# Samsung/tf-fast-rnnt

Hardware: AMD Instinct MI355X
Metric: rnnt_loss_pruned_fwd_bwd_throughput (higher is better)
Workload: dtype f32; 1 GPU; c3: rnnt_loss_pruned fwd+bwd step, B=32/GPU T=1000 S=200 C=500 s_range=5, regular, full boundary, first pass rnnt_loss_simple; global_batch=32, am_pruned=broadcast view

## Files before the change

### tf-fast-rnnt_amd/csrc/ftr_common.h

```cpp
#pragma once
#include <hip/hip_runtime.h>
#include <stdint.h>
#include <stdio.h>
#include <stdarg.h>
#include "../../include/ftr.h"

namespace ftr {

void set_error(const char* fmt, ...);
void clear_error();

inline int check_launch(const char* what) {
  hipError_t e = hipGetLastError();
  if (e != hipSuccess) {
    set_error("%s: launch failed: %s", what, hipGetErrorString(e));
    return FTR_ERR_LAUNCH;
  }
  return FTR_OK;
}

__global__ void zero_words_kernel(uint32_t* __restrict__ p, size_t n);
__global__ void copy_words_kernel(uint32_t* __restrict__ dst, const uint32_t* __restrict__ src, size_t n);
inline int zero_words(void* p, size_t n_words, hipStream_t st, const char* what) {
  if (n_words == 0) return FTR_OK;
// ... 43 lines not shown
  v = fmaxf(v, dpp_take<0x112, 0xf, 0xf>(ninf, v));
  v = fmaxf(v, dpp_take<0x114, 0xf, 0xe>(ninf, v));
  v = fmaxf(v, dpp_take<0x118, 0xf, 0xc>(ninf, v));
  v = fmaxf(v, dpp_take<0x142, 0xa, 0xf>(ninf, v));
  v = fmaxf(v, dpp_take<0x143, 0xc, 0xf>(ninf, v));
  return __builtin_bit_cast(float, __builtin_amdgcn_readlane(__builtin_bit_cast(int, v), 63));
}

struct Shift { float cx2, cy2; };
__device__ __forceinline__ bool shift_sample_ok(float v) { return v > -1.0e4f && v < 1.0e4f; }
template <bool MOD>
__device__ __forceinline__ Shift shift_from_sums(float sumx, float nx, float sumy, float ny, int Sn, int Tn) {
  const float steps = MOD ? (float)(Tn - 1) : (float)(Sn - 1 + Tn - 1);
  float f = steps > 0.0f ? (float)(Sn - 1) / steps : 0.5f;
  f = fminf(fmaxf(f, 1.0e-3f), 1.0f - 1.0e-3f);
  const float mx = nx > 0.0f ? sumx / nx : 0.0f, my = ny > 0.0f ? sumy / ny : 0.0f;
  Shift s;
  s.cx2 = mx * kLog2e - __builtin_amdgcn_logf(f);
  s.cy2 = my * kLog2e - __builtin_amdgcn_logf(1.0f - f);
  return s;
}
template <bool MOD>
__device__ __forceinline__ double shift_total(const Shift s, int Sn, int Tn) {
  const int nx = Sn - 1, ny = MOD ? (Tn - 1) - (Sn - 1) : (Tn - 1);
  return (double)nx * (double)s.cx2 + (double)ny * (double)s.cy2;
}

struct Bound { int sb, tb, se, te; };
__device__ __forceinline__ Bound load_boundary(const int32_t* __restrict__ boundary, int b, int S, int T) {
  Bound r;
  if (boundary) {
    r.sb = max(boundary[4 * b + 0], 0); r.tb = max(boundary[4 * b + 1], 0);
    r.se = min(boundary[4 * b + 2], S); r.te = min(boundary[4 * b + 3], T);
  } else { r.sb = 0; r.tb = 0; r.se = S; r.te = T; }
  return r;
}

__device__ __forceinline__ float softplus(float v) { return fmaxf(v, 0.0f) + log1pf(expf(-fabsf(v))); }
__device__ __forceinline__ void hat_logprobs(float xb, float xs, float Z, bool sym_is_blank, float* vx, float* vy) {
  *vy = -softplus(-xb);
  *vx = sym_is_blank ? -INFINITY : (xs - Z) - softplus(xb);
}
__device__ __forceinline__ void hat_sigmoids(float xb, float* sp, float* sn) {
  const float e = expf(-fabsf(xb)), big = 1.0f / (1.0f + e), small = e / (1.0f + e);
  *sp = xb >= 0.0f ? big : small;
  *sn = xb >= 0.0f ? small : big;
}

}

namespace ftr {
int mi_plain_fwd(const float* px, const float* py, const int32_t* boundary, float* p, float* ans, int B, int S, int T, int modified, hipStream_t st);
int mi_plain_bwd(const float* px, const float* py, const int32_t* boundary, const float* p, float* p_grad, float* px_grad, float* py_grad, float* ans_grad, int overwrite, int B, int S, int T, int modified, hipStream_t st);
int mi_bidir_fwd(const float* px, const float* py, const int32_t* boundary, float* ws, size_t ws_floats, int flags, float* ans, int B, int S, int T, int modified, hipStream_t st);
int mi_bidir_bwd(const int32_t* boundary, const float* ws, size_t ws_floats, int flags, float* px_grad, float* py_grad, float* ans_grad, int overwrite, int B, int S, int T, int modified, hipStream_t st, const float* ans = nullptr, float* loss_out = nullptr, int loss_code = 0);
int mi_bidir_ws_init(float* ws, size_t ws_floats, int B, int S, int T, hipStream_t st);
int mi_bidir_status(const float* ws, size_t ws_floats, int B, int S, int T, int* status_host, long long* dirty_host, hipStream_t st);
size_t mi_bidir_workspace_floats(int B, int S, int T);
size_t mi_bidir_handoff_floats(int B, int S, int T);
size_t mi_viterbi_workspace_bytes(int B, int S, int T);
int mi_viterbi(const float* px, const float* py, const int32_t* boundary, void* ws, size_t ws_bytes, float* score, int32_t* frames, int B, int S, int T, int modified, hipStream_t st);
int cummin_i32(const int32_t* in, int32_t* out, int rows, int cols, hipStream_t st);
int prune_ranges(const float* px_grad, const float* py_grad, const int32_t* boundary, int32_t* ranges, int32_t* s_begin, int B, int S, int T, int T1, int r, hipStream_t st);
int do_pruning(const float* am, const float* lm, const int32_t* ranges, float* am_p, float* lm_p, int B, int T, int S1, int C, int r, hipStream_t st);
size_t do_pruning_bwd_workspace_bytes(int B, int T, int S1, int C, int r);
int do_pruning_bwd_ws(const float* g_am_p, const float* g_lm_p, const int32_t* ranges, float* d_am, float* d_lm, int B, int T, int S1, int C, int r, void* ws, size_t ws_bytes, hipStream_t st);
int do_pruning_bwd(const float* g_am_p, const float* g_lm_p, const int32_t* ranges, float* d_am, float* d_lm, int B, int T, int S1, int C, int r, hipStream_t st);
int pruned_logprobs_fwd(const float* logits, const int32_t* symbols, const int32_t* ranges, const int32_t* boundary, int blank, double delay_penalty, float* lse, float* px, float* py, int B, int T, int S, int C, int r, int modified, int hat, hipStream_t st);
int pruned_logprobs_bwd(const float* logits, const int32_t* symbols, const int32_t* ranges, const int32_t* boundary, int blank, const float* lse, const float* gpx, const float* gpy, Scale scale, float* glogits, int B, int T, int S, int C, int r, int modified, int hat, hipStream_t st);
int simple_rowmax_exp(const float* x, float* probs, float* rowmax, float* rowsum, const float* dotvec, float* dot, size_t rows, int C, hipStream_t st);
int simple_rowmax_exp_pair(const float* x1, float* probs1, float* rowmax1, size_t rows1, const float* x2, float* probs2, float* rowmax2, size_t rows2, int C, hipStream_t st);
int simple_rowdot(const float* x, const float* v, float* dot, size_t rows, int C, hipStream_t st);
size_t simple_colsum_workspace_floats(size_t rows, int C);
int simple_colsum_weighted(const float* x, const float* w, float* out, float* ws, size_t ws_floats, size_t rows, int C, hipStream_t st);
int simple_logprobs_fwd(const float* am, const float* lm, const int32_t* symbols, const float* prod, const float* am_max, const float* lm_max, const int32_t* boundary, int blank, double delay_penalty, const float* lmonly_norm, const float* amonly_norm, const float* ulog, float cs, float ls, float as, float* px, float* py, int B, int T, int S, int C, int modified, hipStream_t st);
int simple_logprobs_bwd_w(const float* gpx, const float* gpy, Scale scale, const float* prod, const int32_t* boundary, float* W, float* rsx, float* rsy, float cs, int B, int T, int S, int modified, hipStream_t st);
int simple_logprobs_bwd_am(const float* gpx, const float* gpy, Scale scale, const float* damp, const float* am_probs, const int32_t* symbols, const int32_t* boundary, int blank, float kdir, const float* uvec, const float* amdot, float as, float* Rout, float* d_am, int B, int T, int S, int C, int modified, hipStream_t st);
int simple_logprobs_bwd_lm(const float* dlmp, const float* lm_probs, const int32_t* symbols, const float* rsx, const float* rsy, int blank, float kdir, const float* arow, const float* invsum, const float* gu, float* d_lm, int B, int S, int C, hipStream_t st);
int simple_fused_supported(int C);
int simple_fused_bwd_supported(int T, int C);
int normalizer_gemm(int kind, const float* x, const float* y, float* out, int B, int T, int S1, int C, hipStream_t st);
int normalizer_gemm_choice(int kind, int B, int T, int S1, int C, int* solution, float* us, float* us_default, int* candidates);
int normalizer_gemm_set_choice(int kind, int B, int T, int S1, int C, int solution);
int simple_fused_fwd(const float* am, const float* lm, const int32_t* symbols, const float* am_probs, const float* lm_probs, const float* am_max, const float* lm_max, const int32_t* boundary, int blank, double delay_penalty, const float* lmonly_norm, const float* amonly_norm, const float* ulog, float cs, float ls, float as, float* px, float* py, float* prod_out, int B, int T, int S, int C, int modified, hipStream_t st);
int simple_fused_bwd_am(const float* gpx, const float* gpy, Scale scale, const float* prod, const float* lm_probs, const float* am_probs, const int32_t* symbols, const int32_t* boundary, int blank, float cs, float kdir, const float* uvec, const float* amdot, float as, float* Rout, float* d_am, int B, int T, int S, int C, int modified, hipStream_t st);
int negated_reduce(const float* ans, int B, int reduction, float* out, hipStream_t st);
int lse_rows(const float* logits, float* lse, size_t rows, int C, int blank, int hat, hipStream_t st);
int mi_band_supported(int T, int S, int r);
int band_ranges_check(const int32_t* ranges, const int32_t* boundary, int* flags, int B, int T, int r, hipStream_t st);
int band_gather(const float* logits, const int32_t* symbols, const int32_t* ranges, const int32_t* boundary, const float* lse, int blank, double delay_penalty, float* pxb, float* pyb, int B, int T, int S, int C, int r, int modified, int hat, hipStream_t st);
size_t mi_band_workspace_floats(int B, int T, int S, int r);
int mi_band_seg_supported(int T, int S, int r);
size_t mi_band_seg_workspace_floats(int B, int T, int S, int r);
int mi_band_seg(const float* pxb, const float* pyb, const int32_t* ranges, const int32_t* boundary, float* ws, size_t ws_floats, float* ans, float* gxb, float* gyb, int B, int T, int S, int r, int modified, hipStream_t st);
int mi_band(const float* pxb, const float* pyb, const int32_t* ranges, const int32_t* boundary, float* ws, size_t ws_floats, float* ans, float* gxb, float* gyb, int B, int T, int S, int r, int modified, hipStream_t st);
int band_grad_banded(const float* logits, const int32_t* symbols, const int32_t* ranges, const int32_t* boundary, int blank, const float* lse, const float* gxb, const float* gyb, Scale scale, float* glogits, int B, int T, int S, int C, int r, int modified, int hat, hipStream_t st);
int selftest(hipStream_t st, int* result_dev);
int debug_stamps(unsigned long long* out16);
int debug_trace(unsigned long long* out, int n);
}
```

### tf-fast-rnnt_amd/csrc/normalizer_gemm.hip

```cpp
#define ROCBLAS_BETA_FEATURES_API 1
#define ROCBLAS_NO_DEPRECATED_WARNINGS 1
#include <rocblas/rocblas.h>

#include <cstdlib>
#include <cstring>
#include <map>
#include <mutex>
#include <tuple>
#include <vector>

#include "ftr_common.h"

namespace ftr {
namespace {

struct Shape {
  int ta, tb, m, n, k, lda, ldb, ldc, batch, device;
  long long sa, sb, sc;
  bool operator<(const Shape& o) const {
    return std::tie(ta, tb, m, n, k, lda, ldb, ldc, batch, device, sa, sb, sc) <
           std::tie(o.ta, o.tb, o.m, o.n, o.k, o.lda, o.ldb, o.ldc, o.batch, o.device, o.sa, o.sb, o.sc);
  }
};
struct Choice {
  int seen = 0;
  bool tuned = false;
  int solution = 0;
  float us = 0.f, us_default = 0.f;
  int candidates = 0;
};

std::mutex g_mu;
std::map<int, rocblas_handle> g_handles;
std::map<Shape, Choice> g_choices;

int tune_mode() {
  const char* e = getenv("FTR_GEMM_TUNE");
  if (!e || !strcmp(e, "second") || !strcmp(e, "auto")) return 2;
  if (!strcmp(e, "first")) return 1;
  return 0;
}

rocblas_status run(rocblas_handle h, const Shape& s, const float* A, const float* B, float* C, rocblas_gemm_algo algo, int sol) {
  const float one = 1.0f, zero = 0.0f;
  return rocblas_gemm_strided_batched_ex(h, (rocblas_operation)s.ta, (rocblas_operation)s.tb, s.m, s.n, s.k, &one, A,
                                         rocblas_datatype_f32_r, s.lda, s.sa, B, rocblas_datatype_f32_r, s.ldb, s.sb, &zero, C,
                                         rocblas_datatype_f32_r, s.ldc, s.sc, C, rocblas_datatype_f32_r, s.ldc, s.sc, s.batch,
                                         rocblas_datatype_f32_r, algo, sol, rocblas_gemm_flags_none);
}

void tune(rocblas_handle h, const Shape& s, const float* A, const float* B, float* C, hipStream_t st, Choice& ch) {
  const float one = 1.0f, zero = 0.0f;
  rocblas_int n = 0;
  auto query = [&](rocblas_int* list, rocblas_int* size) {
    return rocblas_gemm_strided_batched_ex_get_solutions(h, (rocblas_operation)s.ta, (rocblas_operation)s.tb, s.m, s.n, s.k, &one, A,
                                                         rocblas_datatype_f32_r, s.lda, s.sa, B, rocblas_datatype_f32_r, s.ldb, s.sb,
                                                         &zero, C, rocblas_datatype_f32_r, s.ldc, s.sc, C, rocblas_datatype_f32_r,
                                                         s.ldc, s.sc, s.batch, rocblas_datatype_f32_r, rocblas_gemm_algo_solution_index,
                                                         rocblas_gemm_flags_none, list, size);
  };
  ch.tuned = true;
  if (query(nullptr, &n) != rocblas_status_success || n <= 0) return;
  std::vector<rocblas_int> sols((size_t)n);
  if (query(sols.data(), &n) != rocblas_status_success) return;
  hipEvent_t e0, e1;
  if (hipEventCreate(&e0) != hipSuccess) return;
  if (hipEventCreate(&e1) != hipSuccess) { (void)hipEventDestroy(e0); return; }
  auto time_one = [&](rocblas_gemm_algo algo, int sol, int reps) -> float {
    if (run(h, s, A, B, C, algo, sol) != rocblas_status_success) return -1.f;
    (void)hipEventRecord(e0, st);
    for (int i = 0; i < reps; ++i)
      if (run(h, s, A, B, C, algo, sol) != rocblas_status_success) return -1.f;
    (void)hipEventRecord(e1, st);
    if (hipEventSynchronize(e1) != hipSuccess) return -1.f;
    float ms = 0.f;
    (void)hipEventElapsedTime(&ms, e0, e1);
    return 1e3f * ms / reps;
  };
  const float def = time_one(rocblas_gemm_algo_standard, 0, 3);
  std::vector<std::pair<float, int>> timed;
  float fastest = 1e30f;
  for (int i = 0; i < n; ++i) {
    const float t = time_one(rocblas_gemm_algo_solution_index, sols[(size_t)i], 1);
    if (t > 0.f) { timed.emplace_back(t, sols[(size_t)i]); fastest = t < fastest ? t : fastest; }
  }
  float best = def > 0.f ? def : 1e30f;
  int best_sol = 0;
  for (const auto& p : timed) {
    if (p.first > 1.15f * fastest) continue;
    const float t = time_one(rocblas_gemm_algo_solution_index, p.second, 4);
    if (t > 0.f && t < 0.97f * best) { best = t; best_sol = p.second; }
  }
  (void)hipEventDestroy(e0);
  (void)hipEventDestroy(e1);
  (void)hipGetLastError();
  ch.solution = best_sol;
  ch.us = best < 1e29f ? best : 0.f;
  ch.us_default = def;
  ch.candidates = (int)timed.size();
}

}

namespace {
bool make_shape(int kind, int B, int T, int S1, int C, int dev, Shape& s) {
  if (kind == 0)
    s = Shape{rocblas_operation_transpose, rocblas_operation_none, T, S1, C, C, C, T, B, dev, (long long)T * C, (long long)S1 * C, (long long)S1 * T};
  else if (kind == 1)
    s = Shape{rocblas_operation_none, rocblas_operation_none, C, S1, T, C, T, C, B, dev, (long long)T * C, (long long)S1 * T, (long long)S1 * C};
  else if (kind == 2)
    s = Shape{rocblas_operation_none, rocblas_operation_transpose, C, T, S1, C, T, C, B, dev, (long long)S1 * C, (long long)S1 * T, (long long)T * C};
  else
    return false;
  return true;
}
}

int normalizer_gemm(int kind, const float* x, const float* y, float* out, int B, int T, int S1, int C, hipStream_t st) {
  if ((size_t)B * T * S1 * C == 0) return FTR_OK;
  int dev = 0;
  if (hipGetDevice(&dev) != hipSuccess) { set_error("normalizer_gemm: hipGetDevice failed"); return FTR_ERR_LAUNCH; }
  Shape s{};
  if (!make_shape(kind, B, T, S1, C, dev, s)) {
    set_error("normalizer_gemm: kind %d is not 0, 1 or 2", kind);
    return FTR_ERR_INVALID_ARG;
  }
  const float *A = y, *Bm = x;
  std::lock_guard<std::mutex> lock(g_mu);
  rocblas_handle& h = g_handles[dev];
  if (!h) {
    if (rocblas_create_handle(&h) != rocblas_status_success) { h = nullptr; set_error("normalizer_gemm: rocblas_create_handle failed"); return FTR_ERR_LAUNCH; }
    (void)rocblas_set_pointer_mode(h, rocblas_pointer_mode_host);
  }
  if (rocblas_set_stream(h, st) != rocblas_status_success) { set_error("normalizer_gemm: rocblas_set_stream failed"); return FTR_ERR_LAUNCH; }
  Choice& ch = g_choices[s];
  ++ch.seen;
  const int mode = tune_mode();
  if (!ch.tuned && mode != 0 && ch.seen >= mode) {
    hipStreamCaptureStatus cap = hipStreamCaptureStatusNone;
    if (hipStreamIsCapturing(st, &cap) == hipSuccess && cap == hipStreamCaptureStatusNone) tune(h, s, A, Bm, out, st, ch);
  }
  rocblas_status rs = ch.solution ? run(h, s, A, Bm, out, rocblas_gemm_algo_solution_index, ch.solution)
                                  : run(h, s, A, Bm, out, rocblas_gemm_algo_standard, 0);
  if (rs != rocblas_status_success && ch.solution) {
    ch.solution = 0;
    rs = run(h, s, A, Bm, out, rocblas_gemm_algo_standard, 0);
  }
  if (rs != rocblas_status_success) { set_error("normalizer_gemm: rocblas_gemm_strided_batched_ex failed with status %d", (int)rs); return FTR_ERR_LAUNCH; }
  return FTR_OK;
}

int normalizer_gemm_choice(int kind, int B, int T, int S1, int C, int* solution, float* us, float* us_default, int* candidates) {
  int dev = 0;
  (void)hipGetDevice(&dev);
  Shape s{};
  if (!make_shape(kind, B, T, S1, C, dev, s)) return 0;
  std::lock_guard<std::mutex> lock(g_mu);
  const auto it = g_choices.find(s);
  if (it == g_choices.end()) return 0;
  if (solution) *solution = it->second.solution;
  if (us) *us = it->second.us;
  if (us_default) *us_default = it->second.us_default;
  if (candidates) *candidates = it->second.tuned ? it->second.candidates : -1;
  return 1;
}

int normalizer_gemm_set_choice(int kind, int B, int T, int S1, int C, int solution) {
  int dev = 0;
  (void)hipGetDevice(&dev);
  Shape s{};
  if (!make_shape(kind, B, T, S1, C, dev, s)) { set_error("normalizer_gemm_set_choice: kind %d is not 0, 1 or 2", kind); return FTR_ERR_INVALID_ARG; }
  std::lock_guard<std::mutex> lock(g_mu);
  Choice& ch = g_choices[s];
  ch.tuned = true;
  ch.solution = solution;
  ch.candidates = 0;
  return FTR_OK;
}

}
```

### tf-fast-rnnt_amd/csrc/prune.hip

```cpp
#include "ftr_common.h"
#include <cstring>
#include <cstdlib>
#include <limits.h>

namespace ftr {
namespace {

__device__ __forceinline__ int wave_incl_min_scan(int v, int lane) {
#pragma unroll
  for (int off = 1; off < 64; off <<= 1) {
    const int t = __shfl_up(v, off, 64);
    if (lane >= off) v = min(v, t);
  }
  return v;
}

__global__ void cummin_kernel(const int32_t* __restrict__ in, int32_t* __restrict__ out, int rows, int cols) {
  const int lane = threadIdx.x & 63;
  const int row = blockIdx.x * (blockDim.x >> 6) + (threadIdx.x >> 6);
  if (row >= rows) return;
  const int32_t* src = in + (size_t)row * cols;
  int32_t* dst = out + (size_t)row * cols;
  int carry = INT_MAX;
  for (int c0 = 0; c0 < cols; c0 += 64) {
// ... 120 lines not shown
        int pad = se - r + 1;
        if (pad < 0) pad = 0;
        s_begin[(size_t)b * T + t] = (t < te - 1) ? best : pad;
      }
    }
    if (c + 1 < NC) __syncthreads();
  }
}

#ifndef FTR_PRUNE_CHK
#define FTR_PRUNE_CHK 64
#endif
template <int R>
__global__ __launch_bounds__(64) void prune_argmax_once_kernel(const float* __restrict__ px_grad, const float* __restrict__ py_grad,
                                         const int32_t* __restrict__ boundary, int32_t* __restrict__ s_begin,
                                         int B, int S, int T, int T1) {
  const int t = blockIdx.x * blockDim.x + threadIdx.x;
  const int b = blockIdx.y;
  if (t >= T) return;
  const int S1 = S + 1;
  const int nwin = S1 - R + 1;
  const float* pyc = py_grad + (size_t)b * S1 * T + t;
  const float* pxc = px_grad + (size_t)b * S * T1 + t;
  constexpr int CHK = FTR_PRUNE_CHK;
  float carry[R];
  float lead = 0.0f, lag = 0.0f;
#pragma unroll
  for (int s = 0; s < R; ++s) { carry[s] = pyc[(size_t)s * T]; }
#pragma unroll
  for (int s = 0; s < R; ++s) lead = lead + carry[s];
  int best = 0;
  float bestv = 0.0f;
  float nv[2][CHK], xv[2][CHK];
  auto fetch = [&](int c0, float (&n)[CHK], float (&x)[CHK]) {
#pragma unroll
    for (int u = 0; u < CHK; ++u) {
      const int s0 = c0 + u;
      n[u] = (s0 + 1 < nwin) ? pyc[(size_t)(s0 + R) * T] : 0.0f;
      x[u] = (s0 > 0 && s0 < nwin) ? pxc[(size_t)(s0 - 1) * T1] : 0.0f;
    }
  };
  auto consume = [&](int c0, const float (&n)[CHK], const float (&x)[CHK]) {
#pragma unroll
    for (int u = 0; u < CHK; ++u) {
      const int s0 = c0 + u;
      const float g = (u < R) ? carry[u < R ? u : 0] : n[u >= R ? u - R : 0];
      if (s0 < nwin) {
        const float blk = lead - lag;
        const float fin = blk - x[u];
        if (s0 == 0 || fin > bestv) { best = s0; bestv = fin; }
        if (s0 + 1 < nwin) {
          lead = lead + n[u];
          lag = lag + g;
        }
      }
    }
#pragma unroll
    for (int i = 0; i < R; ++i) carry[i] = n[CHK - R + i];
  };
  fetch(0, nv[0], xv[0]);
  for (int c0 = 0; c0 < nwin; c0 += 2 * CHK) {
    if (c0 + CHK < nwin) fetch(c0 + CHK, nv[1], xv[1]);
    consume(c0, nv[0], xv[0]);
    if (c0 + CHK < nwin) {
      if (c0 + 2 * CHK < nwin) fetch(c0 + 2 * CHK, nv[0], xv[0]);
      consume(c0 + CHK, nv[1], xv[1]);
    }
  }
  const int se = boundary[4 * b + 2], te = boundary[4 * b + 3];
  int pad = se - R + 1;
  if (pad < 0) pad = 0;
  s_begin[(size_t)b * T + t] = (t < te - 1) ? best : pad;
}

__device__ __forceinline__ int wave_incl_suffix_min(int v, int lane) {
#pragma unroll
  for (int off = 1; off < 64; off <<= 1) {
    const int t = __shfl_down(v, off, 64);
    if (lane + off < 64) v = min(v, t);
  }
  return v;
}

__global__ void prune_adjust_kernel(const int32_t* __restrict__ s_begin, int32_t* __restrict__ ranges, int B,
                                    int T, int r_out, int r_con) {
  const int lane = threadIdx.x & 63;
  const int b = blockIdx.x * (blockDim.x >> 6) + (threadIdx.x >> 6);
  if (b >= B) return;
  constexpr int PER = 16, SB = 64 * PER;
  const int32_t* x = s_begin + (size_t)b * T;
  int carry1 = INT_MAX, carry2 = INT_MAX;
  for (int base = ((T - 1) / SB) * SB; base >= 0; base -= SB) {
    const int t0 = base + lane * PER;
    int v[PER];
#pragma unroll
    for (int i = 0; i < PER; ++i) v[i] = (t0 + i < T) ? x[t0 + i] : INT_MAX;
#pragma unroll
    for (int i = PER - 2; i >= 0; --i) v[i] = min(v[i], v[i + 1]);
    int incl = wave_incl_suffix_min(v[0], lane);
    int right = __shfl_down(incl, 1, 64);
    right = (lane == 63) ? carry1 : min(right, carry1);
    carry1 = min(__shfl(incl, 0, 64), carry1);
#pragma unroll
    for (int i = 0; i < PER; ++i) {
      const int t = t0 + i;
      v[i] = (t < T) ? -(min(v[i], right) - (r_con - 1) * t) : INT_MAX;
    }
#pragma unroll
    for (int i = PER - 2; i >= 0; --i) v[i] = min(v[i], v[i + 1]);
    incl = wave_incl_suffix_min(v[0], lane);
    right = __shfl_down(incl, 1, 64);
    right = (lane == 63) ? carry2 : min(right, carry2);
    carry2 = min(__shfl(incl, 0, 64), carry2);
#pragma unroll
    for (int i = 0; i < PER; ++i) {
      const int t = t0 + i;
      if (t < T) {
        const int z = max(min(v[i], right), 0);
        const int sb = -(z - (r_con - 1) * t);
        int32_t* dst = ranges + ((size_t)b * T + t) * r_out;
        for (int k = 0; k < r_out; ++k) dst[k] = sb + k;
      }
    }
  }
}

template <bool VEC>
__global__ __launch_bounds__(128) void do_pruning_kernel(const float* __restrict__ am, const float* __restrict__ lm,
                                                         const int32_t* __restrict__ ranges, float* __restrict__ am_p,
                                                         float* __restrict__ lm_p, int T, int S1, int C, int r) {
  const bool copy_am = am_p != nullptr;
  size_t bt = blockIdx.x;
  if ((gridDim.x & 7u) == 0) bt = (size_t)(blockIdx.x & 7u) * (gridDim.x >> 3) + (blockIdx.x >> 3);
  const size_t b = bt / T;
  const int32_t* rg = ranges + bt * r;
  const float* lmb = lm + b * S1 * C;
  float* ao = am_p + bt * r * C;
  float* lo = lm_p + bt * r * C;
  if (VEC) {
    const int n4 = C >> 2;
    const f4u* arow = reinterpret_cast<const f4u*>(am + bt * C);
    for (int c4 = threadIdx.x; c4 < n4; c4 += 128) {
      f4 a = {0.0f, 0.0f, 0.0f, 0.0f};
      if (copy_am) a = arow[c4];
      for (int k0 = 0; k0 < r; k0 += 8) {
        f4 l[8];
#pragma unroll
        for (int u = 0; u < 8; ++u)
          if (k0 + u < r) l[u] = reinterpret_cast<const f4u*>(lmb + (size_t)min(max(rg[k0 + u], 0), S1 - 1) * C)[c4];
#pragma unroll
        for (int u = 0; u < 8; ++u)
          if (k0 + u < r) {
            if (copy_am) __builtin_nontemporal_store(a, reinterpret_cast<f4u*>(ao + (size_t)(k0 + u) * C) + c4);
            __builtin_nontemporal_store(l[u], reinterpret_cast<f4u*>(lo + (size_t)(k0 + u) * C) + c4);
          }
      }
    }
  } else {
    for (int c = threadIdx.x; c < C; c += 128) {
      const float a = copy_am ? am[bt * C + c] : 0.0f;
      for (int k = 0; k < r; ++k) {
        if (copy_am) ao[(size_t)k * C + c] = a;
        lo[(size_t)k * C + c] = lmb[(size_t)min(max(rg[k], 0), S1 - 1) * C + c];
      }
    }
  }
}

template <bool VEC>
__global__ void do_pruning_bwd_am_kernel(const float* __restrict__ g_am_p, float* __restrict__ d_am, int C, int r,
                                         size_t total) {
  const int per_row = VEC ? (C >> 2) : C;
  for (size_t i = (size_t)blockIdx.x * blockDim.x + threadIdx.x; i < total; i += (size_t)gridDim.x * blockDim.x) {
    const size_t bt = i / per_row;
    const int c = (int)(i - bt * per_row);
    if (VEC) {
      f4 acc = {0.f, 0.f, 0.f, 0.f};
      for (int k = 0; k < r; ++k) acc += reinterpret_cast<const f4u*>(g_am_p + (bt * r + k) * C)[c];
      reinterpret_cast<f4u*>(d_am + bt * C)[c] = acc;
    } else {
      float acc = 0.f;
      for (int k = 0; k < r; ++k) acc += g_am_p[(bt * r + k) * C + c];
      d_am[bt * C + c] = acc;
    }
  }
}

template <bool VEC>
__global__ void do_pruning_bwd_lm_kernel(const float* __restrict__ g_lm_p, const int32_t* __restrict__ ranges,
                                         float* __restrict__ d_lm, int T, int S1, int C, int r) {
  extern __shared__ int lds_list[];
  const int s = blockIdx.x, b = blockIdx.y;
  const int n = T * r;
  const int32_t* rg = ranges + (size_t)b * n;
  const int lane = threadIdx.x;
  int count = 0;
  const unsigned long long lt = (1ull << lane) - 1ull;
  const bool vec_ok = ((reinterpret_cast<uintptr_t>(rg) & 15) == 0);
  constexpr int UN = 8;
  for (int base = 0; base < n; base += 256 * UN) {
    int v[UN][4];
#pragma unroll
    for (int u = 0; u < UN; ++u) {
      const int i0 = base + 256 * u + 4 * lane;
      if (vec_ok && i0 + 3 < n) {
// ... 323 lines not shown
          }
        }
        __syncthreads();
        if (wv == 0) {
#pragma unroll
          for (int q = 0; q < 4; ++q) {
            const int c4 = lane + 64 * q;
            if (cb + c4 < n4) tot[q] += RED_WAVES == 4 ? (acc[q] + sums[c4]) + (sums[256 + c4] + sums[512 + c4]) : acc[q] + sums[c4];
          }
        }
      } else if (wv == 0) {
#pragma unroll
        for (int q = 0; q < 4; ++q) tot[q] += acc[q];
      }
      if (last) break;
      __syncthreads();
    }
    if (wv == 0) {
#pragma unroll
      for (int q = 0; q < 4; ++q) {
        const int c4 = cb + lane + 64 * q;
        if (c4 < n4) reinterpret_cast<f4u*>(out)[c4] = tot[q];
      }
    }
    __syncthreads();
  }
}

inline int seg_frames(int B, int T) {
  const char* e = getenv("FTR_PRUNE_SEG");
  const int forced = e ? atoi(e) : 0;
  if (forced >= 4) return forced;
  const long long per = ((long long)B * T + 255) / 256;
  int seg = 16;
  while (seg < per && seg < 128) seg <<= 1;
  return seg;
}
constexpr int kSegMaxR = 16;

}

int do_pruning_bwd(const float* g_am_p, const float* g_lm_p, const int32_t* ranges, float* d_am, float* d_lm, int B,
                   int T, int S1, int C, int r, hipStream_t st) {
  if ((size_t)B * T * C == 0) return FTR_OK;
  const int threads = 256;
  if ((C & 3) == 0) {
    const size_t total = (size_t)B * T * (C >> 2);
    hipLaunchKernelGGL(do_pruning_bwd_am_kernel<true>, dim3((unsigned)((total + threads - 1) / threads)), dim3(threads), 0, st, g_am_p, d_am, C, r, total);
  } else {
    const size_t total = (size_t)B * T * C;
    hipLaunchKernelGGL(do_pruning_bwd_am_kernel<false>, dim3((unsigned)((total + threads - 1) / threads)), dim3(threads), 0, st, g_am_p, d_am, C, r, total);
  }
  int rc = check_launch("do_pruning_bwd_am");
  if (rc != FTR_OK) return rc;
  const size_t lds = sizeof(int) * (size_t)T * r;
  if (lds > 150 * 1024) { set_error("do_pruning_bwd: T*s_range = %d too large for the LDS row list", T * r); return FTR_ERR_UNSUPPORTED; }
  const bool vec = (C & 3) == 0;
  if (lds > 64 * 1024) {
    hipError_t e = vec ? hipFuncSetAttribute(reinterpret_cast<const void*>(do_pruning_bwd_lm_kernel<true>), hipFuncAttributeMaxDynamicSharedMemorySize, (int)lds)
                       : hipFuncSetAttribute(reinterpret_cast<const void*>(do_pruning_bwd_lm_kernel<false>), hipFuncAttributeMaxDynamicSharedMemorySize, (int)lds);
    if (e != hipSuccess) { set_error("do_pruning_bwd: cannot reserve LDS: %s", hipGetErrorString(e)); return FTR_ERR_LAUNCH; }
  }
  if (vec) hipLaunchKernelGGL(do_pruning_bwd_lm_kernel<true>, dim3(S1, B), dim3(64), lds, st, g_lm_p, ranges, d_lm, T, S1, C, r);
  else hipLaunchKernelGGL(do_pruning_bwd_lm_kernel<false>, dim3(S1, B), dim3(64), lds, st, g_lm_p, ranges, d_lm, T, S1, C, r);
  return check_launch("do_pruning_bwd_lm");
}

int cummin_i32(const int32_t* in, int32_t* out, int rows, int cols, hipStream_t st) {
  if (rows == 0 || cols == 0) return FTR_OK;
  const int waves_per_block = 4;
  hipLaunchKernelGGL(cummin_kernel, dim3((rows + waves_per_block - 1) / waves_per_block),
                     dim3(64 * waves_per_block), 0, st, in, out, rows, cols);
  return check_launch("cummin_i32");
}

int prune_ranges(const float* px_grad, const float* py_grad, const int32_t* boundary, int32_t* ranges,
                 int32_t* s_begin, int B, int S, int T, int T1, int r, hipStream_t st) {
  if (B == 0 || T == 0) return FTR_OK;
  const int threads = 64;
  const dim3 grid((T + threads - 1) / threads, B);
#define FTR_ARGMAX_ONCE(R) case R: hipLaunchKernelGGL(prune_argmax_once_kernel<R>, grid, dim3(threads), 0, st, px_grad, py_grad, boundary, s_begin, B, S, T, T1); break;
  const int nwin = S + 1 - r + 1;
  static const bool split_off = getenv("FTR_PRUNE_ARGMAX_SPLIT") && !strcmp(getenv("FTR_PRUNE_ARGMAX_SPLIT"), "0");
  if (nwin > ftr::kSplitQ && (size_t)((T + 63) / 64) * B <= 768 && !split_off) {
    const int nc = (nwin + ftr::kSplitQ - 1) / ftr::kSplitQ;
    const int nw = nc < 8 ? nc : 8;
    hipLaunchKernelGGL(prune_argmax_split_kernel, dim3((T + 63) / 64, B), dim3(64 * nw), 0, st, px_grad, py_grad, boundary, s_begin, B, S, T, T1, r);
  } else
  switch (r) {
    FTR_ARGMAX_ONCE(1) FTR_ARGMAX_ONCE(2) FTR_ARGMAX_ONCE(3) FTR_ARGMAX_ONCE(4) FTR_ARGMAX_ONCE(5) FTR_ARGMAX_ONCE(6)
    FTR_ARGMAX_ONCE(7) FTR_ARGMAX_ONCE(8) FTR_ARGMAX_ONCE(9) FTR_ARGMAX_ONCE(10) FTR_ARGMAX_ONCE(11) FTR_ARGMAX_ONCE(12)
    FTR_ARGMAX_ONCE(13) FTR_ARGMAX_ONCE(14) FTR_ARGMAX_ONCE(15) FTR_ARGMAX_ONCE(16)
    default: hipLaunchKernelGGL(prune_argmax_kernel, grid, dim3(threads), 0, st, px_grad, py_grad, boundary, s_begin, B, S, T, T1, r);
  }
#undef FTR_ARGMAX_ONCE
  int rc = check_launch("prune_argmax");
  if (rc != FTR_OK) return rc;
  const int r_con = (T1 == T) ? 2 : r;
  hipLaunchKernelGGL(prune_adjust_kernel, dim3(B), dim3(64), 0, st, s_begin, ranges, B, T, r, r_con);
  return check_launch("prune_adjust");
}

int do_pruning(const float* am, const float* lm, const int32_t* ranges, float* am_p, float* lm_p, int B, int T, int S1,
               int C, int r, hipStream_t st) {
  const size_t frames = (size_t)B * T;
  if (frames == 0 || C == 0 || r == 0) return FTR_OK;
  if (frames > 0x7fffffffull) { set_error("do_pruning: B*T = %zu exceeds the grid limit", frames); return FTR_ERR_UNSUPPORTED; }
  if ((C & 3) == 0) hipLaunchKernelGGL(do_pruning_kernel<true>, dim3((unsigned)frames), dim3(128), 0, st, am, lm, ranges, am_p, lm_p, T, S1, C, r);
  else hipLaunchKernelGGL(do_pruning_kernel<false>, dim3((unsigned)frames), dim3(128), 0, st, am, lm, ranges, am_p, lm_p, T, S1, C, r);
  return check_launch("do_pruning");
}

size_t do_pruning_bwd_workspace_bytes(int B, int T, int S1, int C, int r) {
  if ((C & 3) != 0 || (size_t)B * T * C == 0 || r <= 0) return 0;
  const int seg = ftr::seg_frames(B, T);
  const size_t nseg = (size_t)(T + seg - 1) / seg;
  const size_t partial = sizeof(float) * (size_t)B * nseg * (2 * (size_t)r) * C;
  return partial + sizeof(int4) * (size_t)B * nseg;
}

int do_pruning_bwd_ws(const float* g_am_p, const float* g_lm_p, const int32_t* ranges, float* d_am, float* d_lm,
                      int B, int T, int S1, int C, int r, void* ws, size_t ws_bytes, hipStream_t st) {
  if ((size_t)B * T * C == 0) return FTR_OK;
  if ((C & 3) != 0 || r <= 0) return do_pruning_bwd(g_am_p, g_lm_p, ranges, d_am, d_lm, B, T, S1, C, r, st);
  const size_t need = do_pruning_bwd_workspace_bytes(B, T, S1, C, r);
  if (!ws || ws_bytes < need || (reinterpret_cast<uintptr_t>(ws) & 15) != 0) {
    set_error("do_pruning_bwd_ws: workspace of %zu bytes (16-byte aligned) required, got %zu", need, ws_bytes);
    return FTR_ERR_INVALID_ARG;
  }
  const int seg = ftr::seg_frames(B, T);
  const int nseg = (T + seg - 1) / seg;
  float* partial = reinterpret_cast<float*>(ws);
  int4* meta = reinterpret_cast<int4*>(partial + (size_t)B * nseg * (2 * (size_t)r) * C);
  const size_t lds = sizeof(int) * (size_t)seg;
  if (r > ftr::kSegMaxR || lds > 60 * 1024 || (size_t)B * nseg * (2 * (size_t)r) >= 0x7fffffffull || (size_t)B * T * r >= 0x7fffffffull)
    return do_pruning_bwd(g_am_p, g_lm_p, ranges, d_am, d_lm, B, T, S1, C, r, st);
  const bool fuse = (g_am_p == g_lm_p);
  if (!fuse) {
    const size_t total = (size_t)B * T * (C >> 2);
    hipLaunchKernelGGL(ftr::do_pruning_bwd_am_kernel<true>, dim3((unsigned)((total + 255) / 256)), dim3(256), 0, st, g_am_p, d_am, C, r, total);
    int rc = check_launch("do_pruning_bwd_am");
    if (rc != FTR_OK) return rc;
  }
#define FTR_SEG(R) case R: \
    if (fuse) hipLaunchKernelGGL((ftr::do_pruning_bwd_seg_kernel<R, true>), dim3(nseg, B), dim3(128), lds, st, g_lm_p, ranges, d_am, d_lm, partial, meta, T, S1, C, seg); \
    else hipLaunchKernelGGL((ftr::do_pruning_bwd_seg_kernel<R, false>), dim3(nseg, B), dim3(128), lds, st, g_lm_p, ranges, d_am, d_lm, partial, meta, T, S1, C, seg); \
    break;
  switch (r) {
    FTR_SEG(1) FTR_SEG(2) FTR_SEG(3) FTR_SEG(4) FTR_SEG(5) FTR_SEG(6) FTR_SEG(7) FTR_SEG(8)
    FTR_SEG(9) FTR_SEG(10) FTR_SEG(11) FTR_SEG(12) FTR_SEG(13) FTR_SEG(14) FTR_SEG(15) FTR_SEG(16)
  }
#undef FTR_SEG
  int rc = check_launch("do_pruning_bwd_seg");
  if (rc != FTR_OK) return rc;
  hipLaunchKernelGGL(ftr::do_pruning_bwd_reduce_kernel, dim3(S1, B), dim3(64 * ftr::RED_WAVES),
                     sizeof(int) * (size_t)((2 * nseg + 3) & ~3) + 3 * 256 * sizeof(float) * 4, st, g_lm_p, ranges, partial, meta, d_lm, T, S1, C, r, seg, nseg);
  return check_launch("do_pruning_bwd_reduce");
}

}
```

Measured before the change: 24060 utterances/s.

## Add native MFMA kernel for kind-1 normalizer GEMM with autotune routing

```diff
diff --git a/tf-fast-rnnt_amd/csrc/ftr_common.h b/tf-fast-rnnt_amd/csrc/ftr_common.h
--- a/tf-fast-rnnt_amd/csrc/ftr_common.h
+++ b/tf-fast-rnnt_amd/csrc/ftr_common.h
@@ -149,6 +149,9 @@
 int normalizer_gemm(int kind, const float* x, const float* y, float* out, int B, int T, int S1, int C, hipStream_t st);
 int normalizer_gemm_choice(int kind, int B, int T, int S1, int C, int* solution, float* us, float* us_default, int* candidates);
 int normalizer_gemm_set_choice(int kind, int B, int T, int S1, int C, int solution);
+int normalizer_mfma_kind1_supported(int T, int C);
+int normalizer_mfma_kind1_fills(int B, int T, int S1, int C);
+int normalizer_mfma_kind1(const float* W, const float* am_probs, float* dlmp, int B, int T, int S1, int C, hipStream_t st);
 int simple_fused_fwd(const float* am, const float* lm, const int32_t* symbols, const float* am_probs, const float* lm_probs, const float* am_max, const float* lm_max, const int32_t* boundary, int blank, double delay_penalty, const float* lmonly_norm, const float* amonly_norm, const float* ulog, float cs, float ls, float as, float* px, float* py, float* prod_out, int B, int T, int S, int C, int modified, hipStream_t st);
 int simple_fused_bwd_am(const float* gpx, const float* gpy, Scale scale, const float* prod, const float* lm_probs, const float* am_probs, const int32_t* symbols, const int32_t* boundary, int blank, float cs, float kdir, const float* uvec, const float* amdot, float as, float* Rout, float* d_am, int B, int T, int S, int C, int modified, hipStream_t st);
 int negated_reduce(const float* ans, int B, int reduction, float* out, hipStream_t st);
diff --git a/tf-fast-rnnt_amd/csrc/normalizer_gemm.hip b/tf-fast-rnnt_amd/csrc/normalizer_gemm.hip
--- a/tf-fast-rnnt_amd/csrc/normalizer_gemm.hip
+++ b/tf-fast-rnnt_amd/csrc/normalizer_gemm.hip
@@ -4,6 +4,7 @@
 
 #include <cstdlib>
 #include <cstring>
+#include <functional>
 #include <map>
 #include <mutex>
 #include <tuple>
@@ -49,7 +50,10 @@
                                          rocblas_datatype_f32_r, algo, sol, rocblas_gemm_flags_none);
 }
 
-void tune(rocblas_handle h, const Shape& s, const float* A, const float* B, float* C, hipStream_t st, Choice& ch) {
+constexpr int kNative = -1;
+
+void tune(rocblas_handle h, const Shape& s, const float* A, const float* B, float* C, hipStream_t st, Choice& ch,
+          const std::function<int()>& native) {
   const float one = 1.0f, zero = 0.0f;
   rocblas_int n = 0;
   auto query = [&](rocblas_int* list, rocblas_int* size) {
@@ -91,6 +95,17 @@
     const float t = time_one(rocblas_gemm_algo_solution_index, p.second, 4);
     if (t > 0.f && t < 0.97f * best) { best = t; best_sol = p.second; }
   }
+  if (native && native() == FTR_OK) {
+    (void)hipEventRecord(e0, st);
+    bool ok = true;
+    for (int i = 0; i < 4 && ok; ++i) ok = native() == FTR_OK;
+    (void)hipEventRecord(e1, st);
+    float ms = 0.f;
+    if (ok && hipEventSynchronize(e1) == hipSuccess && hipEventElapsedTime(&ms, e0, e1) == hipSuccess) {
+      const float t = 1e3f * ms / 4;
+      if (t < 0.97f * best) { best = t; best_sol = kNative; }
+    }
+  }
   (void)hipEventDestroy(e0);
   (void)hipEventDestroy(e1);
   (void)hipGetLastError();
@@ -125,6 +140,14 @@
     set_error("normalizer_gemm: kind %d is not 0, 1 or 2", kind);
     return FTR_ERR_INVALID_ARG;
   }
+  std::function<int()> native;
+  if (kind == 1 && normalizer_mfma_kind1_supported(T, C)) {
+    const char* e = getenv("FTR_GEMM_ROUTE");
+    const int route = !e || !strcmp(e, "auto") ? 0 : !strcmp(e, "native") ? 1 : -1;
+    if (route == 1) return normalizer_mfma_kind1(x, y, out, B, T, S1, C, st);
+    if (route == 0 && normalizer_mfma_kind1_fills(B, T, S1, C))
+      native = [=]() { return normalizer_mfma_kind1(x, y, out, B, T, S1, C, st); };
+  }
   const float *A = y, *Bm = x;
   std::lock_guard<std::mutex> lock(g_mu);
   rocblas_handle& h = g_handles[dev];
@@ -138,8 +161,10 @@
   const int mode = tune_mode();
   if (!ch.tuned && mode != 0 && ch.seen >= mode) {
     hipStreamCaptureStatus cap = hipStreamCaptureStatusNone;
-    if (hipStreamIsCapturing(st, &cap) == hipSuccess && cap == hipStreamCaptureStatusNone) tune(h, s, A, Bm, out, st, ch);
-  }
+    if (hipStreamIsCapturing(st, &cap) == hipSuccess && cap == hipStreamCaptureStatusNone) tune(h, s, A, Bm, out, st, ch, native);
+  }
+  if (native && (!ch.tuned || ch.solution == kNative)) return native();
+  if (ch.solution == kNative) ch.solution = 0;
   rocblas_status rs = ch.solution ? run(h, s, A, Bm, out, rocblas_gemm_algo_solution_index, ch.solution)
                                   : run(h, s, A, Bm, out, rocblas_gemm_algo_standard, 0);
   if (rs != rocblas_status_success && ch.solution) {
diff --git a/tf-fast-rnnt_amd/csrc/normalizer_mfma.hip b/tf-fast-rnnt_amd/csrc/normalizer_mfma.hip
--- /dev/null
+++ b/tf-fast-rnnt_amd/csrc/normalizer_mfma.hip
@@ -0,0 +1,202 @@
+#include "ftr_common.h"
+
+namespace ftr {
+namespace {
+
+typedef float v4f __attribute__((ext_vector_type(4)));
+constexpr int kNT = 64;
+constexpr int kKC = 16;
+constexpr int kWaves = 4;
+
+template <int MBN>
+__host__ __device__ constexpr size_t kind1_lds_bytes() {
+  return sizeof(float) * 2 * (size_t)MBN * 4 * 64 * 4;
+}
+
+template <int MBN>
+__global__ __launch_bounds__(256, 1) void normalizer_kind1_kernel(const float* __restrict__ W, const float* __restrict__ P,
+                                                                  float* __restrict__ out, int M, int N, int K, int mtiles,
+                                                                  int ntiles) {
+  extern __shared__ __attribute__((aligned(16))) float smem[];
+  const unsigned total = gridDim.x, lin = blockIdx.x;
+  const unsigned j = (total & 7u) == 0 ? (lin & 7u) * (total >> 3) + (lin >> 3) : lin;
+  const int nt = j % ntiles, mt = (j / ntiles) % mtiles, b = j / (ntiles * mtiles);
+  const int m0 = mt * 16 * MBN, n0 = nt * kNT;
+  const int lane = threadIdx.x & 63;
+  const int wave = __builtin_amdgcn_readfirstlane(threadIdx.x >> 6);
+  const int q = lane >> 4, l16 = lane & 15;
+
+  const int nc = (K + kKC - 1) / kKC;
+  const int c_begin = wave * nc / kWaves, c_end = (wave + 1) * nc / kWaves;
+
+  const float* Wb = W + (size_t)b * M * K;
+  const float* Pb = P + (size_t)b * K * N;
+  const int pcol = min(n0 + 4 * l16, N - 4);
+  auto wrow = [&](int mb) { return min(m0 + 16 * mb + l16, M - 1) * K; };
+
+  struct Frag { f4 w[MBN]; f4 p[4]; };
+  auto load = [&](int c, Frag& f) {
+    const int kq = c * kKC + 4 * q;
+#pragma unroll
+    for (int mb = 0; mb < MBN; ++mb) f.w[mb] = *reinterpret_cast<const f4u*>(Wb + (unsigned)(wrow(mb) + kq));
+#pragma unroll
+    for (int s = 0; s < 4; ++s) f.p[s] = *reinterpret_cast<const f4u*>(Pb + (unsigned)((kq + s) * N + pcol));
+  };
+  auto load_tail = [&](int c, Frag& f) {
+    const int kq = c * kKC + 4 * q;
+    const bool kin = kq < K;
+    const int kqc = kin ? kq : K - 4;
+#pragma unroll
+    for (int mb = 0; mb < MBN; ++mb) {
+      const f4 v = *reinterpret_cast<const f4u*>(Wb + (unsigned)(wrow(mb) + kqc));
+      f.w[mb] = kin ? v : f4{0.f, 0.f, 0.f, 0.f};
+    }
+#pragma unroll
+    for (int s = 0; s < 4; ++s) {
+      const f4 v = *reinterpret_cast<const f4u*>(Pb + (unsigned)((kqc + s) * N + pcol));
+      f.p[s] = kin ? v : f4{0.f, 0.f, 0.f, 0.f};
+    }
+  };
+
+  v4f acc[MBN][4];
+#pragma unroll
+  for (int mb = 0; mb < MBN; ++mb)
+#pragma unroll
+    for (int e = 0; e < 4; ++e) acc[mb][e] = v4f{0.f, 0.f, 0.f, 0.f};
+
+  auto compute = [&](const Frag& f) {
+#pragma unroll
+    for (int s = 0; s < 4; ++s)
+#pragma unroll
+      for (int mb = 0; mb < MBN; ++mb)
+#pragma unroll
+        for (int e = 0; e < 4; ++e) acc[mb][e] = __builtin_amdgcn_mfma_f32_16x16x4f32(f.p[s][e], f.w[mb][s], acc[mb][e], 0, 0, 0);
+  };
+
+  const int c_full = min(c_end, K / kKC);
+  if (c_begin < c_full) {
+    Frag cur;
+    load(c_begin, cur);
+    for (int c = c_begin; c < c_full; ++c) {
+      Frag nxt;
+      load(min(c + 1, c_full - 1), nxt);
+      __builtin_amdgcn_sched_barrier(0);
+      compute(cur);
+      __builtin_amdgcn_sched_barrier(0);
+      cur = nxt;
+#pragma unroll
+      for (int mb = 0; mb < MBN; ++mb) asm volatile("" : "+v"(cur.w[mb]));
+#pragma unroll
+      for (int s = 0; s < 4; ++s) asm volatile("" : "+v"(cur.p[s]));
+    }
+  }
+  if (c_full < c_end) {
+    Frag f;
+    load_tail(c_full, f);
+    compute(f);
+  }
+
+  constexpr int PART = MBN * 4 * 64 * 4;
+  auto park = [&](float* dst) {
+#pragma unroll
+    for (int mb = 0; mb < MBN; ++mb)
+#pragma unroll
+      for (int e = 0; e < 4; ++e) *reinterpret_cast<v4f*>(dst + ((mb * 4 + e) * 64 + lane) * 4) = acc[mb][e];
+  };
+  auto take = [&](const float* src) {
+#pragma unroll
+    for (int mb = 0; mb < MBN; ++mb) {
+#pragma unroll
+      for (int e = 0; e < 4; ++e) acc[mb][e] += *reinterpret_cast<const v4f*>(src + ((mb * 4 + e) * 64 + lane) * 4);
+      __builtin_amdgcn_sched_barrier(0);
+    }
+  };
+  if (wave >= 2) park(smem + (wave - 2) * PART);
+  __syncthreads();
+  if (wave < 2) take(smem + wave * PART);
+  __syncthreads();
+  if (wave == 1) park(smem);
+  __syncthreads();
+  if (wave != 0) return;
+  take(smem);
+
+  float* ob = out + (size_t)b * M * N;
+#pragma unroll
+  for (int mb = 0; mb < MBN; ++mb) {
+    const int m = m0 + 16 * mb + l16;
+    if (m >= M) continue;
+#pragma unroll
+    for (int r = 0; r < 4; ++r) {
+      const int n = n0 + 16 * q + 4 * r;
+      if (n < N) *reinterpret_cast<f4u*>(ob + (size_t)m * N + n) = f4{acc[mb][0][r], acc[mb][1][r], acc[mb][2][r], acc[mb][3][r]};
+    }
+  }
+}
+
+template <int MBN>
+int launch_kind1(const float* W, const float* P, float* out, int B, int M, int N, int K, int mtiles, hipStream_t st) {
+  static bool raised = false;
+  if (!raised) {
+    if (hipFuncSetAttribute(reinterpret_cast<const void*>(normalizer_kind1_kernel<MBN>), hipFuncAttributeMaxDynamicSharedMemorySize,
+                            (int)kind1_lds_bytes<MBN>()) != hipSuccess) {
+      (void)hipGetLastError();
+      set_error("normalizer_gemm: cannot raise the dynamic LDS limit");
+      return FTR_ERR_LAUNCH;
+    }
+    raised = true;
+  }
+  const int ntiles = (N + kNT - 1) / kNT;
+  const size_t total = (size_t)B * mtiles * ntiles;
+  hipLaunchKernelGGL(normalizer_kind1_kernel<MBN>, dim3((unsigned)total), dim3(256), kind1_lds_bytes<MBN>(), st, W, P, out, M, N,
+                     K, mtiles, ntiles);
+  return check_launch("normalizer_gemm (kind 1, MFMA)");
+}
+
+int cu_count() {
+  static int n = 0;
+  if (!n) {
+    int dev = 0, v = 0;
+    (void)hipGetDevice(&dev);
+    n = (hipDeviceGetAttribute(&v, hipDeviceAttributeMultiprocessorCount, dev) == hipSuccess && v > 0) ? v : 256;
+  }
+  return n;
+}
+
+long long kind1_plan(int B, int S1, int C, int& mbn, int& mtiles) {
+  const int nb = (S1 + 15) / 16, ntiles = (C + kNT - 1) / kNT, cus = cu_count();
+  long long best_cost = -1, best_wgs = 0;
+  for (int m : {13, 10, 7, 4}) {
+    const long long mt = (nb + m - 1) / m, wgs = (long long)B * ntiles * mt;
+    const long long cost = ((wgs + cus - 1) / cus) * m;
+    if (best_cost < 0 || cost < best_cost) { best_cost = cost; best_wgs = wgs; mbn = m; mtiles = (int)mt; }
+  }
+  return best_wgs;
+}
+
+}
+
+int normalizer_mfma_kind1_supported(int T, int C) { return (T >= 4 && C >= 4 && T % 4 == 0 && C % 4 == 0) ? 1 : 0; }
+
+static bool kind1_offsets_fit(int T, int S1, int C) { return (long long)S1 * T < (1LL << 31) && (long long)T * C < (1LL << 31); }
+
+int normalizer_mfma_kind1_fills(int B, int T, int S1, int C) {
+  int mbn = 0, mtiles = 0;
+  return kind1_offsets_fit(T, S1, C) && kind1_plan(B, S1, C, mbn, mtiles) >= cu_count() && mbn >= 7 ? 1 : 0;
+}
+
+int normalizer_mfma_kind1(const float* W, const float* am_probs, float* dlmp, int B, int T, int S1, int C, hipStream_t st) {
+  if (!normalizer_mfma_kind1_supported(T, C) || !kind1_offsets_fit(T, S1, C)) {
+    set_error("normalizer_gemm: T = %d, S1 = %d, C = %d is outside the MFMA kernel's domain", T, S1, C);
+    return FTR_ERR_UNSUPPORTED;
+  }
+  int best = 13, mtiles = 1;
+  if (kind1_plan(B, S1, C, best, mtiles) > 0x7fffffffLL) { set_error("normalizer_gemm: grid too large"); return FTR_ERR_UNSUPPORTED; }
+  switch (best) {
+    case 13: return launch_kind1<13>(W, am_probs, dlmp, B, S1, C, T, mtiles, st);
+    case 10: return launch_kind1<10>(W, am_probs, dlmp, B, S1, C, T, mtiles, st);
+    case 7: return launch_kind1<7>(W, am_probs, dlmp, B, S1, C, T, mtiles, st);
+    default: return launch_kind1<4>(W, am_probs, dlmp, B, S1, C, T, mtiles, st);
+  }
+}
+
+}
```

New measurement: 24060 utterances/s (median of 5 runs). Within noise of the previous version (-0.0%).

## Parallelize prune_adjust suffix scans across a 512-thread block with coalesced range writes

Applied to the files above, without the earlier changes.

```diff
diff --git a/tf-fast-rnnt_amd/csrc/prune.hip b/tf-fast-rnnt_amd/csrc/prune.hip
--- a/tf-fast-rnnt_amd/csrc/prune.hip
+++ b/tf-fast-rnnt_amd/csrc/prune.hip
@@ -226,8 +226,8 @@
   return v;
 }
 
-__global__ void prune_adjust_kernel(const int32_t* __restrict__ s_begin, int32_t* __restrict__ ranges, int B,
-                                    int T, int r_out, int r_con) {
+__global__ void prune_adjust_wave_kernel(const int32_t* __restrict__ s_begin, int32_t* __restrict__ ranges, int B,
+                                         int T, int r_out, int r_con) {
   const int lane = threadIdx.x & 63;
   const int b = blockIdx.x * (blockDim.x >> 6) + (threadIdx.x >> 6);
   if (b >= B) return;
@@ -265,6 +265,66 @@
         int32_t* dst = ranges + ((size_t)b * T + t) * r_out;
         for (int k = 0; k < r_out; ++k) dst[k] = sb + k;
       }
+    }
+  }
+}
+
+constexpr int kAdjThreads = 512, kAdjPer = 4, kAdjSB = kAdjThreads * kAdjPer;
+__global__ __launch_bounds__(kAdjThreads) void prune_adjust_kernel(const int32_t* __restrict__ s_begin, int32_t* __restrict__ ranges,
+                                                                   int B, int T, int r_out, int r_con) {
+  constexpr int NW = kAdjThreads / 64, PER = kAdjPer, SB = kAdjSB;
+  __shared__ int wt1[NW], wt2[NW];
+  __shared__ int sbv[SB];
+  const int lane = threadIdx.x & 63, wave = threadIdx.x >> 6;
+  const int b = blockIdx.x;
+  const int32_t* x = s_begin + (size_t)b * T;
+  int carry1 = INT_MAX, carry2 = INT_MAX;
+  auto block_right = [&](int first, int* wt, int& total) -> int {
+    const int incl = wave_incl_suffix_min(first, lane);
+    if (lane == 0) wt[wave] = incl;
+    __syncthreads();
+    int rw = INT_MAX;
+    total = INT_MAX;
+#pragma unroll
+    for (int w = 0; w < NW; ++w) {
+      const int m = wt[w];
+      total = min(total, m);
+      if (w > wave) rw = min(rw, m);
+    }
+    const int right = __shfl_down(incl, 1, 64);
+    return (lane == 63) ? rw : min(right, rw);
+  };
+  for (int base = ((T - 1) / SB) * SB; base >= 0; base -= SB) {
+    const int t0 = base + (int)threadIdx.x * PER;
+    int v[PER];
+#pragma unroll
+    for (int i = 0; i < PER; ++i) v[i] = (t0 + i < T) ? x[t0 + i] : INT_MAX;
+#pragma unroll
+    for (int i = PER - 2; i >= 0; --i) v[i] = min(v[i], v[i + 1]);
+    int total;
+    int right = min(block_right(v[0], wt1, total), carry1);
+    carry1 = min(total, carry1);
+#pragma unroll
+    for (int i = 0; i < PER; ++i) {
+      const int t = t0 + i;
+      v[i] = (t < T) ? -(min(v[i], right) - (r_con - 1) * t) : INT_MAX;
+    }
+#pragma unroll
+    for (int i = PER - 2; i >= 0; --i) v[i] = min(v[i], v[i + 1]);
+    right = min(block_right(v[0], wt2, total), carry2);
+    carry2 = min(total, carry2);
+#pragma unroll
+    for (int i = 0; i < PER; ++i) {
+      const int t = t0 + i;
+      const int z = max(min(v[i], right), 0);
+      sbv[threadIdx.x * PER + i] = -(z - (r_con - 1) * t);
+    }
+    __syncthreads();
+    const int n = min(SB, T - base) * r_out;
+    int32_t* dst = ranges + ((size_t)b * T + base) * r_out;
+    for (int i = threadIdx.x; i < n; i += kAdjThreads) {
+      const int f = i / r_out;
+      dst[i] = sbv[f] + (i - f * r_out);
     }
   }
 }
@@ -754,6 +814,8 @@
 #define FTR_ARGMAX_ONCE(R) case R: hipLaunchKernelGGL(prune_argmax_once_kernel<R>, grid, dim3(threads), 0, st, px_grad, py_grad, boundary, s_begin, B, S, T, T1); break;
   const int nwin = S + 1 - r + 1;
   static const bool split_off = getenv("FTR_PRUNE_ARGMAX_SPLIT") && !strcmp(getenv("FTR_PRUNE_ARGMAX_SPLIT"), "0");
+  const char* route_env = getenv("FTR_PRUNE_ROUTE");
+  const bool legacy = route_env && !strcmp(route_env, "legacy");
   if (nwin > ftr::kSplitQ && (size_t)((T + 63) / 64) * B <= 768 && !split_off) {
     const int nc = (nwin + ftr::kSplitQ - 1) / ftr::kSplitQ;
     const int nw = nc < 8 ? nc : 8;
@@ -769,7 +831,8 @@
   int rc = check_launch("prune_argmax");
   if (rc != FTR_OK) return rc;
   const int r_con = (T1 == T) ? 2 : r;
-  hipLaunchKernelGGL(prune_adjust_kernel, dim3(B), dim3(64), 0, st, s_begin, ranges, B, T, r, r_con);
+  if (legacy) hipLaunchKernelGGL(prune_adjust_wave_kernel, dim3(B), dim3(64), 0, st, s_begin, ranges, B, T, r, r_con);
+  else hipLaunchKernelGGL(prune_adjust_kernel, dim3(B), dim3(ftr::kAdjThreads), 0, st, s_begin, ranges, B, T, r, r_con);
   return check_launch("prune_adjust");
 }
 
```

After: 23970 utterances/s before, 24010 utterances/s after, median of 3. No clear change (+0.2%).
